# TheaQG/DiffusionModelsCustom

Measured on NVIDIA B200. Metric: samples_per_s_T1000_ddpm_sampling, higher is better.
Workload: dtype fp16 operands, fp32 accumulate (fp32 state/update)

## Files before the change

### diffusionmodelscustom_b200/_native.py

```python
from __future__ import annotations

import ctypes as C
import os

_PKG = os.path.dirname(os.path.abspath(__file__))
LIB_PATH = os.environ.get("B2D_LIB") or os.path.join(_PKG, "libb200ddpm.so")

FAMILY_R, FAMILY_D = 0, 1
INTERP_MODES = {"bicubic": 0, "bilinear": 1, "nearest": 2}

SYMBOLS = ["b2d_last_error", "b2d_abi_version", "b2d_create", "b2d_destroy", "b2d_load_weights", "b2d_set_schedule",
           "b2d_set_conditioning", "b2d_forward", "b2d_sample", "b2d_sample_host", "b2d_last_launch_count", "b2d_debug_read", "b2d_profile_step",
           "b2d_op_conv2d", "b2d_op_layernorm", "b2d_op_attention", "b2d_op_attn_block", "b2d_op_attn_block_out", "b2d_op_instnorm", "b2d_op_posterior_update", "b2d_saturation_count", "b2d_debug_attn_trace", "b2d_ensemble_run",
           "b2d_op_noise_image", "b2d_op_weighted_mse", "b2d_op_eval_daily", "b2d_op_eval_pixel", "b2d_op_histogram", "b2d_encoder_forward", "b2d_decoder_forward", "b2d_op_final_layer",
           "b2d_set_timesteps", "b2d_op_ddim_update"]


class Config(C.Structure):
    _fields_ = [(n, C.c_int32) for n in ("family", "img_size", "max_batch", "c_hr", "c_out", "has_lsm", "has_topo",
                                         "cond_channels", "num_classes", "n_heads", "attn_ff", "debug_simt_conv",
                                         "interp_mode", "stem_embedding")]


class Tensor(C.Structure):
    _fields_ = [("name", C.c_char_p), ("data", C.c_void_p), ("ndim", C.c_int32), ("shape", C.c_int64 * 4)]


class OpProfile(C.Structure):
    _fields_ = [("name", C.c_char * 48), ("klass", C.c_char * 24), ("flops", C.c_double), ("bytes", C.c_double),
                ("ms", C.c_double)]


class NativeError(RuntimeError):
    pass


_lib = None


def lib():
    global _lib
    if _lib is None:
        if not os.path.exists(LIB_PATH):
            raise NativeError(f"{LIB_PATH} is missing: build it with `python -m diffusionmodelscustom_b200.build` "
                              "(there is no fallback path)")
        L = C.CDLL(LIB_PATH)
        L.b2d_last_error.restype = C.c_char_p
        L.b2d_abi_version.restype = C.c_int
        L.b2d_create.argtypes = [C.POINTER(Config), C.POINTER(C.c_void_p)]
        L.b2d_destroy.argtypes = [C.c_void_p]
        L.b2d_destroy.restype = None
        L.b2d_load_weights.argtypes = [C.c_void_p, C.POINTER(Tensor), C.c_int32]
        L.b2d_set_schedule.argtypes = [C.c_void_p, C.c_void_p, C.c_void_p, C.c_void_p, C.c_int32]
        L.b2d_set_conditioning.argtypes = [C.c_void_p, C.c_void_p, C.c_void_p, C.c_void_p, C.c_int32, C.c_int32,
                                           C.c_void_p, C.c_int32, C.c_void_p]
        L.b2d_forward.argtypes = [C.c_void_p, C.c_void_p, C.c_void_p, C.c_void_p, C.c_int32, C.c_void_p]
        L.b2d_sample.argtypes = [C.c_void_p, C.c_void_p, C.c_void_p, C.c_uint64, C.c_uint64, C.c_float, C.c_int32,
                                 C.c_void_p]
        L.b2d_sample_host.argtypes = [C.c_void_p, C.c_void_p, C.c_void_p, C.c_void_p, C.c_void_p, C.c_int32, C.c_int32,
                                      C.c_void_p, C.c_void_p, C.c_uint64, C.c_uint64, C.c_float, C.c_int32]
        L.b2d_last_launch_count.argtypes = [C.c_void_p]
        L.b2d_last_launch_count.restype = C.c_int64
        L.b2d_debug_read.argtypes = [C.c_void_p, C.c_char_p, C.c_void_p, C.c_int64, C.POINTER(C.c_int32), C.POINTER(C.c_int32)]
        L.b2d_profile_step.argtypes = [C.c_void_p, C.c_void_p, C.c_void_p, C.c_int32, C.c_int32, C.POINTER(OpProfile),
                                       C.c_int32, C.POINTER(C.c_int32)]
        L.b2d_op_conv2d.argtypes = [C.c_void_p] * 5 + [C.c_int32, C.c_void_p] + [C.c_int32] * 12 + [C.c_void_p]
        L.b2d_op_layernorm.argtypes = [C.c_void_p] * 4 + [C.c_int32, C.c_int32, C.c_void_p]
        L.b2d_op_attention.argtypes = [C.c_void_p, C.c_void_p] + [C.c_int32] * 4 + [C.c_void_p]
        L.b2d_op_attn_block.argtypes = [C.c_void_p] * 5 + [C.c_int32] * 4 + [C.c_void_p]
        L.b2d_op_attn_block_out.argtypes = [C.c_void_p] * 7 + [C.c_int32] * 5 + [C.c_void_p]
        L.b2d_op_instnorm.argtypes = [C.c_void_p, C.c_void_p, C.c_void_p, C.c_int32, C.c_void_p, C.c_void_p] + \
                                     [C.c_int32] * 3 + [C.c_void_p]
        L.b2d_op_final_layer.argtypes = [C.c_void_p] * 4 + [C.c_int32] * 4 + [C.c_void_p]
        L.b2d_op_posterior_update.argtypes = [C.c_void_p] * 6 + [C.c_int32, C.c_int32, C.c_int64, C.c_uint64, C.c_uint64,
                                                                 C.c_float, C.c_void_p]
        L.b2d_set_timesteps.argtypes = [C.c_void_p, C.c_void_p, C.c_int32, C.c_float]
        L.b2d_op_ddim_update.argtypes = [C.c_void_p] * 4 + [C.c_int32] * 3 + [C.c_float, C.c_int32, C.c_int64, C.c_uint64,
                                                              C.c_uint64, C.c_float, C.c_void_p]
        L.b2d_op_noise_image.argtypes = [C.c_void_p] * 6 + [C.c_int32, C.c_int64, C.c_uint64, C.c_uint64, C.c_float, C.c_void_p]
        L.b2d_op_weighted_mse.argtypes = [C.c_void_p] * 3 + [C.c_float, C.c_float, C.c_void_p, C.c_int64, C.c_void_p]
        L.b2d_op_eval_daily.argtypes = [C.c_void_p] * 4 + [C.c_int32, C.c_int64, C.c_void_p]
        L.b2d_op_eval_pixel.argtypes = [C.c_void_p] * 5 + [C.c_int32, C.c_int64, C.c_void_p]
        L.b2d_op_histogram.argtypes = [C.c_void_p, C.c_int64, C.c_float, C.c_float, C.c_int32, C.c_void_p, C.c_void_p]
        L.b2d_encoder_forward.argtypes = [C.c_void_p, C.c_void_p, C.c_void_p, C.POINTER(C.c_void_p), C.c_int32, C.c_void_p]
        L.b2d_decoder_forward.argtypes = [C.c_void_p, C.POINTER(C.c_void_p), C.c_void_p, C.c_void_p, C.c_int32, C.c_void_p]
        L.b2d_saturation_count.argtypes = [C.c_int32]
        L.b2d_saturation_count.restype = C.c_uint32
        if L.b2d_abi_version() != 1:
            raise NativeError("libb200ddpm.so ABI version mismatch")
        _lib = L
    return _lib


def check(rc: int):
    if rc != 0:
        raise NativeError(f"b200ddpm error {rc}: {lib().b2d_last_error().decode(errors='replace')}")


def ptr(t):
    return None if t is None else t.data_ptr()
```

### diffusionmodelscustom_b200/csrc/b200ddpm.cu

```cuda
#include "../../include/b200ddpm.h"

#include <chrono>
#include <cmath>
#include <cstring>
#include <functional>
#include <map>
#include <memory>
#include <vector>

#include "attention.cuh"
#include "attention_tc.cuh"
#include "attention_tc2.cuh"
#include "attention_tc3.cuh"
#include "attention_tc3d32.cuh"
#include "attention_tc6.cuh"
#include "attention_tc8.cuh"
#include "attn_block.cuh"
#include "common.cuh"
#include "conv.cuh"
#include "conv_persist.cuh"
#include "elementwise.cuh"
#include "evalops.cuh"
#include "gemm_stream.cuh"
#include "norm_fused.cuh"
#include "tail_tc.cuh"

namespace b2d {
thread_local Status g_status;
int g_pdl_enabled = getenv("B2D_NO_PDL") ? 0 : 1;

static inline cudaStream_t as_stream(void* s) { return reinterpret_cast<cudaStream_t>(s); }

struct HostTensor {
    std::vector<float> v;
    std::vector<int64_t> shape;
    size_t numel() const { return v.size(); }
};

static inline uint16_t f2h(float f) {
    const float c = f > 65504.0f ? 65504.0f : (f < -65504.0f ? -65504.0f : f);
    const __half h = __float2half_rn(c);
    uint16_t u;
    memcpy(&u, &h, 2);
    return u;
}

typedef std::function<int(cudaStream_t)> OpFn;
struct Op {
    std::string name;
    std::string klass;
    double flops = 0;
    double bytes = 0;
    OpFn fn;
    bool side = false;
    bool join = false;
    int operator()(cudaStream_t st) const { return fn(st); }
};
struct OpList {
    std::vector<Op> v;
    Op pending;
    void meta(const std::string& name, const std::string& klass, double flops, double bytes) {
        pending.name = name; pending.klass = klass; pending.flops = flops; pending.bytes = bytes;
    }
    void push_back(OpFn f) {
        pending.fn = std::move(f);
        v.push_back(pending);
        pending = Op();
    }
};

struct EnsembleRes;
void ensemble_release(EnsembleRes* r);
struct Handle {
    b2d_config cfg{};
    int num_sms = 148;
    std::vector<void*> allocs;
    std::vector<void*> prog_allocs;
    bool in_prog = false;
// ... 642 lines not shown
        const std::string r0 = "l" + std::to_string(li) + "b0", r1 = "l" + std::to_string(li) + "b1";
        f16* t1 = bd.act(n_out);
        f16* b0 = bd.act(n_out);
        f16* pre = bd.act(n_out);
        const f16* identity = cur;
        const int stride = (li > 1) ? 2 : 1;
        if (li > 1) {
            f16* ds = bd.act(n_out);
            ops.pending.side = true;
            bd.conv(cur, hin, hin, cin, ds, cout, 1, 2, 0, false, r0 + ".ds", nullptr, nullptr, 0, 0);
            identity = ds;
        }
        bd.conv(cur, hin, hin, cin, t1, cout, 3, stride, 1, false, r0 + ".c1", nullptr, nullptr, 0, 1);
        ops.pending.join = (li > 1);
        bd.conv(t1, hout, hout, cout, b0, cout, 3, 1, 1, false, r0 + ".c2", identity, nullptr, 0, 1);
        bd.conv(b0, hout, hout, cout, t1, cout, 3, 1, 1, false, r1 + ".c1", nullptr, nullptr, 0, 1);
        bd.conv(t1, hout, hout, cout, pre, cout, 3, 1, 1, false, r1 + ".c2", b0, temb + TEMB_ENC_OFF[li], TS, 1);
        fmap[li] = bd.act(n_out);
        bd.attention(pre, hout, cout, "ea" + std::to_string(li), fmap[li], 0);
        h->taps["pre" + std::to_string(li + 1)] = {pre, cout, hout};
        h->taps["fmap" + std::to_string(li + 1)] = {fmap[li], cout, hout};
        cur = fmap[li];
        cin = cout;
    }
    h->dec_begin_op = (int)ops.v.size();
    for (int i = 0; i < 5; ++i) h->fmaps[i] = {fmap[i], ENC_CH[i], s[i + 1]};
    const f16* dcur = fmap[4];
    for (int i = 0; i < 4; ++i) {
        const int ci = DEC_IN[i], co = DEC_OUT[i];
        const int hin = s[5 - i], hout = s[4 - i];
        const std::string r = "d" + std::to_string(i);
        f16* up = bd.act((size_t)B * hout * hout * ci);
        bd.conv(dcur, hin, hin, ci, up, ci, 1, 1, 0, true, r + ".up", nullptr, nullptr, 0, 0);
        if (!bd.instnorm_fused(up, nullptr, nullptr, 0, up, hout, ci)) {
            float* st1 = bd.stats_slice(ci);
            bd.plane_stats(up, hout, ci, st1);
            bd.instnorm_apply(up, st1, nullptr, nullptr, 0, up, hout, ci);
        }
        f16* cv = bd.act((size_t)B * hout * hout * co);
        bd.conv(up, hout, hout, ci, cv, co, 3, 1, 1, false, r + ".conv", nullptr, nullptr, 0, 0);
        f16* pre = bd.act((size_t)B * hout * hout * co);
        if (!bd.instnorm_fused(cv, fmap[3 - i], temb + TEMB_DEC_OFF[i], TS, pre, hout, co)) {
            float* st2 = bd.stats_slice(co);
            bd.plane_stats(cv, hout, co, st2);
            bd.instnorm_apply(cv, st2, fmap[3 - i], temb + TEMB_DEC_OFF[i], TS, pre, hout, co);
        }
        f16* dout = bd.act((size_t)B * hout * hout * co);
        bd.attention(pre, hout, co, "da" + std::to_string(i), dout, 1 );
        h->taps["dec" + std::to_string(i) + "_pre"] = {pre, co, hout};
        h->taps["dec" + std::to_string(i)] = {dout, co, hout};
        dcur = dout;
    }
    h->temb_free_op = (int)ops.v.size();
    {
        f16* up = bd.act((size_t)B * H * H * 64);
        bd.conv(dcur, s[1], s[1], 64, up, 64, 1, 1, 0, true, "final.up", nullptr, nullptr, 0, 0);
        float* st = bd.stats_slice(64);
        bd.plane_stats(up, H, 64, st);
        Handle* hh = h;
        const float* tw = bd.W<float>("tail.w");
        const float* tb = bd.W<float>("tail.b");
        const float* twk = bd.W<float>("tail.wk");
        const int cout = c.c_out, Hh = H;
        ops.meta("final.conv", "tail_conv", 2.0 * B * Hh * Hh * 576 * cout, (double)B * Hh * Hh * (64 * 2 + 4 * cout));
        static const bool no_tc_tail = getenv("B2D_NO_TC_TAIL") != nullptr;
        auto ttp = std::make_shared<TailTcPlan>();
        const bool tc_tail = tail_tc_supported(Hh, Hh, cout) && !no_tc_tail;
        if (tc_tail && tail_tc_plan_build(*ttp, up, B, Hh, Hh) != 0) return g_status.code ? g_status.code : fail(-1, "tail plan failed");
        ops.push_back([=](cudaStream_t s2) {
            dim3 grid((Hh + 31) / 32, (Hh + 7) / 8, B);
            static const bool simt_tail = getenv("B2D_SIMT_TAIL") != nullptr;
            if (tc_tail)
                return tail_tc_launch(*ttp, st, twk, tb, hh->cur_eps, Hh, Hh, s2);
            if (cout <= 8 && !simt_tail)
                B2D_CUDA(launch_k(tail_mma_kernel, dim3(grid), dim3(256), TAILM_SMEM, s2, up, st, twk, tb, hh->cur_eps, Hh, Hh, cout));
            else
                B2D_CUDA(launch_k(tail_conv_kernel, dim3(grid), dim3(256), TAIL_SMEM, s2, up, st, tw, tb, hh->cur_eps, Hh, Hh, cout));
            B2D_CUDA(cudaGetLastError());
            return 0;
        });
    }
    if (bd.err) return g_status.code ? g_status.code : fail(-1, "program build failed");
    if (h->stats_floats > STATS_CAPACITY_PER_SAMPLE * (size_t)c.max_batch) return fail(-1, "internal: stats buffer too small");
    h->step_ops.swap(ops.v);
    h->prog_B = B;
    return 0;
}

template <typename K>
static int set_carveout(K kern) {
    B2D_CUDA(cudaFuncSetAttribute(kern, cudaFuncAttributePreferredSharedMemoryCarveout, cudaSharedmemCarveoutMaxShared));
    return 0;
}
static int init_uniform_carveout() {
    static bool done = false;
    if (done || getenv("B2D_NO_CARVEOUT")) return 0;
    B2D_TRY(set_carveout(conv_tc_kernel<64, 4>));
    B2D_TRY(set_carveout(conv_tc_kernel<64, 8>));
    B2D_TRY(set_carveout(conv_tc_kernel<128, 3>));
    B2D_TRY(set_carveout(conv_tc_kernel<128, 6>));
    B2D_TRY(set_carveout(conv_simt_kernel));
    B2D_TRY(set_carveout(layernorm_rows_kernel<64>));
    B2D_TRY(set_carveout(layernorm_rows_kernel<128>));
    B2D_TRY(set_carveout(layernorm_rows_kernel<256>));
    B2D_TRY(set_carveout(layernorm_rows_kernel<512>));
    B2D_TRY(set_carveout(flash_attn_kernel<16>));
    B2D_TRY(set_carveout(flash_attn_kernel<32>));
    B2D_TRY(set_carveout(flash_attn_kernel<64>));
    B2D_TRY(set_carveout(flash_attn_kernel<128>));
    B2D_TRY(set_carveout(attn_small_d_kernel<2>));
    B2D_TRY(set_carveout(attn_small_d_kernel<4>));
    B2D_TRY(set_carveout(attn_small_d_kernel<8>));
    B2D_TRY(set_carveout(attn_tc_kernel));
    B2D_TRY(set_carveout(attn_tc2_kernel<0>));
    B2D_TRY(set_carveout(attn_tc2_kernel<1>));
    B2D_TRY(set_carveout(attn_tc2_kernel<2>));
    B2D_TRY(set_carveout(attn_tc2_kernel<3>));
    B2D_TRY(set_carveout(attn_tc2_kernel<4>));
// ... 136 lines not shown
        B2D_TRY(h->alloc(&h->d_ddim_coef, T + 1));
        h->ddim_cap = T + 1;
    }
    std::vector<int> tau(h->ddim_tau);
    tau.resize(S + 2, 0);
    std::vector<float4> coef(S);
    for (int k = 0; k < S; ++k)
        coef[k] = ddim_coefficients(h->h_alpha_hat[tau[k]], k + 1 < S ? h->h_alpha_hat[tau[k + 1]] : 1.0f, h->ddim_eta);
    B2D_CUDA(cudaMemcpy(h->d_ddim_tau, tau.data(), tau.size() * sizeof(int), cudaMemcpyHostToDevice));
    B2D_CUDA(cudaMemcpy(h->d_ddim_coef, coef.data(), coef.size() * sizeof(float4), cudaMemcpyHostToDevice));
    h->ddim_dirty = false;
    return 0;
}

}

using namespace b2d;

extern "C" {

const char* b2d_last_error(void) { return g_status.msg.c_str(); }
int b2d_abi_version(void) { return B2D_ABI_VERSION; }

int b2d_create(const b2d_config* cfg, b2d_handle** out) {
    B2D_CHECK(cfg && out, "null argument");
    B2D_CHECK(cfg->family == B2D_FAMILY_R || cfg->family == B2D_FAMILY_D, "unknown family");
    B2D_CHECK(is_pow2(cfg->img_size) && cfg->img_size >= 32 && cfg->img_size <= 128, "img_size must be 32, 64 or 128");
    B2D_CHECK(cfg->max_batch >= 1, "max_batch must be positive");
    B2D_CHECK(cfg->c_hr >= 1 && cfg->c_out >= 1, "channel counts must be positive");
    int dev = 0, ndev = 0;
    cudaError_t e = cudaGetDeviceCount(&ndev);
    if (e != cudaSuccess || ndev == 0)
        return fail(-2, "no CUDA device: this library has no CPU fallback (" + std::string(cudaGetErrorString(e)) + ")");
    B2D_CUDA(cudaGetDevice(&dev));
    cudaDeviceProp prop;
    B2D_CUDA(cudaGetDeviceProperties(&prop, dev));
    B2D_CHECK(prop.major == 10, "b200ddpm kernels are compiled for sm_100a only");
    auto* h = new b2d_handle();
    h->cfg = *cfg;
    if (h->cfg.n_heads <= 0) h->cfg.n_heads = 4;
    h->num_sms = prop.multiProcessorCount;
    int rc = 0;
    do {
        if ((rc = conv_tc_init_attrs())) break;
        if ((rc = conv_tcp_init_attrs())) break;
        if ((rc = flash_attn_init_attrs())) break;
        if ((rc = attn_tc_init_attrs())) break;
        if ((rc = attn_tc2_init_attrs())) break;
        if ((rc = attn_tc3_init_attrs())) break;
        if ((rc = attn_tc5_init_attrs())) break;
        if ((rc = attn_tc6_init_attrs())) break;
        if ((rc = attn_tc8_init_attrs())) break;
        if ((rc = tail_tc_init_attrs())) break;
        if ((rc = gemm_stream_init_attrs())) break;
        if ((rc = attn_block_init_attrs())) break;
        if ((rc = norm_fused_init_attrs())) break;
        if ((rc = init_uniform_carveout())) break;
        const int B = cfg->max_batch, H = cfg->img_size;
        const size_t n = (size_t)B * cfg->c_hr * H * H, plane = (size_t)H * H;
        if ((rc = init_batch_buffers(h))) break;
        if ((rc = h->alloc(&h->d_x_work, n))) break;
        if ((rc = h->alloc(&h->d_job, 1))) break;
        if (cfg->family == B2D_FAMILY_R) {
            if (cfg->has_lsm && (rc = h->alloc(&h->d_lsm_stage, (size_t)B * plane))) break;
            if (cfg->has_topo && (rc = h->alloc(&h->d_topo_stage, (size_t)B * plane))) break;
        }
        h->cond_stage_elems = (size_t)B * std::max(cfg->cond_channels, 1) * plane;
        if ((rc = h->alloc(&h->d_cond_stage, h->cond_stage_elems))) break;
        if (cudaMallocHost(reinterpret_cast<void**>(&h->h_y_pinned), (size_t)B * sizeof(int)) != cudaSuccess) {
            rc = fail(-2, "pinned label staging allocation failed");
            break;
        }
    } while (0);
    if (rc) {
        delete h;
        return rc;
    }
    *out = h;
    return 0;
}

void b2d_destroy(b2d_handle* h) { delete h; }

int b2d_load_weights(b2d_handle* h, const b2d_tensor* tensors, int32_t n) {
    B2D_CHECK(h && tensors && n > 0, "null argument");
    B2D_CHECK(!h->weights_loaded, "weights already loaded on this handle (create a new handle to reload)");
    h->sd.clear();
    for (int i = 0; i < n; ++i) {
        const b2d_tensor& t = tensors[i];
        B2D_CHECK(t.name && t.data && t.ndim >= 0 && t.ndim <= 4, "malformed tensor entry");
        HostTensor ht;
        size_t numel = 1;
        for (int d = 0; d < t.ndim; ++d) {
            ht.shape.push_back(t.shape[d]);
            numel *= (size_t)t.shape[d];
        }
        ht.v.assign(t.data, t.data + numel);
        h->sd[t.name] = std::move(ht);
    }
    int rc = (h->cfg.family == B2D_FAMILY_R) ? pack_family_r(h) : pack_family_d(h);
    h->sd.clear();
    if (rc) return rc;
    h->weights_loaded = true;
    return 0;
}

// ... 543 lines not shown
    float* stats = ws;
    float* partial = ws + n_stats;
    unsigned int* counters = reinterpret_cast<unsigned int*>(ws + n_stats + n_part);
    cudaMemsetAsync(counters, 0, n_cnt * 4, st);
    dim3 grid(nslab, ngrp, B);
    B2D_CUDA(launch_k(plane_stats_kernel, dim3(grid), dim3(256), 0, st, (const f16*)x, partial, counters, stats, HW, C, 256));
    const size_t total8 = (size_t)B * HW * C / 8;
    const int blocks = (int)std::min<size_t>((total8 + 255) / 256, (size_t)148 * 16);
    B2D_CUDA(launch_k(instnorm_apply_kernel, dim3(blocks), dim3(256), 0, st, (const f16*)x, stats, (const f16*)skip, vec, vec_stride, (f16*)y, HW, C,
                                                  total8));
    cudaError_t e = cudaGetLastError();
    cudaStreamSynchronize(st);
    cudaFree(ws);
    B2D_CUDA(e);
    return 0;
}

int b2d_op_final_layer(const void* x, const float* w, const float* bias, float* out, int32_t B, int32_t H, int32_t W,
                       int32_t use_mma_sync, void* stream) {
    cudaStream_t st = as_stream(stream);
    B2D_CHECK(x && w && bias && out && B >= 1 && H >= 1 && W >= 1, "bad argument");
    const int HW = H * W, C = 64;
    const int nslab = (HW + 255) / 256;
    float* ws = nullptr;
    const size_t n_stats = (size_t)B * C * 2, n_part = (size_t)B * nslab * 128, n_cnt = (size_t)B;
    B2D_CUDA(cudaMalloc(&ws, (n_stats + n_part + n_cnt) * 4));
    float* stats = ws;
    float* partial = ws + n_stats;
    unsigned int* counters = reinterpret_cast<unsigned int*>(ws + n_stats + n_part);
    cudaMemsetAsync(counters, 0, n_cnt * 4, st);
    int rc = 0;
    do {
        cudaError_t e = launch_k(plane_stats_kernel, dim3(nslab, 1, B), dim3(256), 0, st, (const f16*)x, partial, counters, stats, HW, C, 256);
        if (e != cudaSuccess) { rc = fail(-2, cudaGetErrorString(e)); break; }
        if (!use_mma_sync && tail_tc_supported(H, W, 1)) {
            if ((rc = tail_tc_init_attrs())) break;
            TailTcPlan pl;
            if ((rc = tail_tc_plan_build(pl, (const f16*)x, B, H, W))) break;
            rc = tail_tc_launch(pl, stats, w, bias, out, H, W, st);
        } else {
            e = cudaFuncSetAttribute(tail_mma_kernel, cudaFuncAttributeMaxDynamicSharedMemorySize, TAILM_SMEM);
            if (e == cudaSuccess)
                e = launch_k(tail_mma_kernel, dim3((W + 31) / 32, (H + 7) / 8, B), dim3(256), TAILM_SMEM, st, (const f16*)x, stats, w, bias, out, H, W, 1);
            if (e != cudaSuccess) rc = fail(-2, cudaGetErrorString(e));
        }
    } while (0);
    cudaError_t e2 = cudaStreamSynchronize(st);
    cudaFree(ws);
    if (rc) return rc;
    B2D_CUDA(e2);
    return 0;
}

int b2d_op_posterior_update(float* x, const float* eps, const float* z, const float* betas, const float* alphas,
                            const float* alpha_hat, int32_t i, int32_t B, int64_t per_sample, uint64_t seed,
                            uint64_t sample_offset, float noise_scale, void* stream) {
    B2D_CHECK(x && eps && betas && alphas && alpha_hat && B >= 1 && per_sample >= 1, "bad argument");
    B2D_CHECK(per_sample % 4 == 0, "per-sample element count must be a multiple of 4 (vectorised update)");
    cudaStream_t st = as_stream(stream);
    struct Scratch { int* step = nullptr; SampleJob* job = nullptr; };
    static thread_local Scratch sc;
    if (!sc.step) {
        B2D_CUDA(cudaMalloc(&sc.step, 16));
        B2D_CUDA(cudaMalloc(&sc.job, sizeof(SampleJob)));
    }
    const size_t n = (size_t)B * per_sample;
    SampleJob job{};
    job.noise = z ? z - (size_t)i * n : nullptr;
    job.seed = seed;
    job.sample_offset = sample_offset;
    job.noise_stride = n;
    job.noise_scale = noise_scale;
    B2D_CUDA(launch_k(set_job_kernel, dim3(1), dim3(32), 0, st, sc.job, job, sc.step + 2, sc.step, (int)i, 0));
    const int blocks = (int)std::min<size_t>((n / 4 + 255) / 256, (size_t)148 * 8);
    B2D_CUDA(launch_k(posterior_update_kernel, dim3(blocks), dim3(256), 0, st, x, eps, sc.job, alphas, betas, alpha_hat, sc.step, nullptr, B, n,
                      (size_t)per_sample));
    B2D_CUDA(cudaGetLastError());
    return 0;
}

int b2d_op_ddim_update(float* x, const float* eps, const float* z_or_null, const float* alpha_hat, int32_t T, int32_t t,
                       int32_t t_prev, float eta, int32_t B, int64_t per_sample, uint64_t seed, uint64_t sample_offset,
                       float noise_scale, void* stream) {
    B2D_CHECK(x && eps && alpha_hat && B >= 1 && per_sample >= 1 && T >= 2, "bad argument");
    B2D_CHECK(per_sample % 4 == 0, "per-sample element count must be a multiple of 4 (vectorised update)");
    B2D_CHECK(t >= 1 && t <= T - 1, "t must lie in [1, T-1]");
    B2D_CHECK(t_prev == -1 || (t_prev >= 1 && t_prev < t), "t_prev must be -1 (final step) or lie in [1, t-1]");
    B2D_CHECK(eta >= 0.f && eta <= 1.f, "eta must lie in [0, 1]");
    cudaStream_t st = as_stream(stream);
    float ah[2] = {0.f, 1.f};
    B2D_CUDA(cudaMemcpyAsync(&ah[0], alpha_hat + t, 4, cudaMemcpyDeviceToHost, st));
    if (t_prev >= 1) B2D_CUDA(cudaMemcpyAsync(&ah[1], alpha_hat + t_prev, 4, cudaMemcpyDeviceToHost, st));
    B2D_CUDA(cudaStreamSynchronize(st));
    const float4 c = ddim_coefficients(ah[0], ah[1], eta);
    struct Scratch { int* step = nullptr; SampleJob* job = nullptr; int* tau = nullptr; float4* coef = nullptr; };
    static thread_local Scratch sc;
    if (!sc.step) {
        B2D_CUDA(cudaMalloc(&sc.step, 16));
        B2D_CUDA(cudaMalloc(&sc.job, sizeof(SampleJob)));
        B2D_CUDA(cudaMalloc(&sc.tau, 16));
        B2D_CUDA(cudaMalloc(&sc.coef, sizeof(float4)));
    }
    const size_t n = (size_t)B * per_sample;
    SampleJob job{};
    job.noise = z_or_null;
    job.seed = seed;
// ... 85 lines not shown
```

### include/b200ddpm.h

```cpp
#ifndef B200DDPM_H
#define B200DDPM_H

#include <stddef.h>
#include <stdint.h>

#ifdef __cplusplus
extern "C" {
#endif

#define B2D_ABI_VERSION 1

typedef struct b2d_handle b2d_handle;

enum { B2D_FAMILY_R = 0,
       B2D_FAMILY_D = 1   };

typedef struct b2d_config {
    int32_t family;
    int32_t img_size;
    int32_t max_batch;
    int32_t c_hr;
    int32_t c_out;
    int32_t has_lsm;
    int32_t has_topo;
// ... 60 lines not shown
typedef struct b2d_ensemble_stats {
    int32_t sub_batches;
    int32_t out_pinned;
    int64_t launches;
    double gather_ms;
    double wall_ms;
} b2d_ensemble_stats;
int b2d_ensemble_run(b2d_handle* h, const b2d_ensemble_job* job, b2d_ensemble_stats* stats);

unsigned int b2d_saturation_count(int32_t reset);

int64_t b2d_last_launch_count(const b2d_handle* h);
typedef struct b2d_op_profile {
    char name[48];
    char klass[24];
    double flops;
    double bytes;
    double ms;
} b2d_op_profile;
int b2d_profile_step(b2d_handle* h, const float* x, const int64_t* t_host, int32_t B, int32_t reps, b2d_op_profile* out,
                     int32_t max_ops, int32_t* n_ops);

int b2d_debug_read(b2d_handle* h, const char* name, float* out_host, int64_t max_elems, int32_t* C_out, int32_t* hw_out);

int b2d_op_noise_image(const float* x0, const int64_t* t_dev, const float* alpha_hat, const float* noise_or_null, float* x_t,
                       float* noise_out, int32_t B, int64_t per_sample, uint64_t seed, uint64_t sample_offset, float noise_scale,
                       void* stream);
int b2d_op_weighted_mse(const float* input, const float* target, const float* sdf_or_null, float max_land_weight,
                        float min_sea_weight, float* out_scalar_dev, int64_t n, void* stream);
int b2d_op_eval_daily(const float* gen, const float* eval, float* mae_out, float* rmse_out, int32_t n_samples, int64_t hw,
                      void* stream);
int b2d_op_eval_pixel(const float* gen, const float* eval, float* mae_out, float* rmse_out, float* bias_out, int32_t n_samples,
                      int64_t hw, void* stream);
int b2d_op_histogram(const float* x, int64_t n, float lo, float hi, int32_t bins, unsigned long long* counts_dev, void* stream);

int b2d_debug_attn_trace(long long* out_host, int32_t max_elems);

int b2d_op_conv2d(const void* in_f16, const void* w_packed_f16, const float* bias, const void* residual_f16,
                  const float* post_add, int32_t post_stride, void* out_f16, int32_t B, int32_t Hi, int32_t Wi,
                  int32_t Cin, int32_t Cout, int32_t R, int32_t S, int32_t stride, int32_t pad, int32_t convt,
                  int32_t act, int32_t impl, void* stream);
int b2d_op_layernorm(const void* x_f16, const float* gamma, const float* beta, void* y_f16, int32_t rows, int32_t C,
                     void* stream);
int b2d_op_attention(const void* qkv_f16, void* o_f16, int32_t B, int32_t L, int32_t C, int32_t heads, void* stream);
int b2d_op_attn_block(const void* x_f16, const void* w_folded_f16, const float* c1, const float* bias, void* o_f16,
                      int32_t B, int32_t L, int32_t C, int32_t heads, void* stream);
int b2d_op_attn_block_out(const void* x_f16, const void* w_folded_f16, const float* c1, const float* bias, const void* wo_f16,
                          const float* out_bias, void* y_f16, int32_t B, int32_t L, int32_t C, int32_t heads,
                          int32_t final_act, void* stream);
int b2d_op_instnorm(const void* x_f16, const void* skip_f16, const float* vec, int32_t vec_stride, void* y_f16,
                    float* stats_ws, int32_t B, int32_t HW, int32_t C, void* stream);
int b2d_op_final_layer(const void* x_f16, const float* w_kmajor, const float* bias, float* out, int32_t B, int32_t H, int32_t W,
                       int32_t use_mma_sync, void* stream);
int b2d_op_posterior_update(float* x, const float* eps, const float* z_or_null, const float* betas, const float* alphas,
                            const float* alpha_hat, int32_t i, int32_t B, int64_t per_sample, uint64_t seed,
                            uint64_t sample_offset, float noise_scale, void* stream);

#ifdef __cplusplus
}
#endif
#endif
```

Before: 26.31.

## Fuse final transposed conv, instance-norm stats and 3x3 tail conv into tcgen05 kernels

Replaces the final 2x-upsampling transposed conv, the instance-norm statistics and the 3x3 output conv with two warp-specialised TMA/tcgen05 kernels. The first pass recomputes the upsampled activations per tile in TMEM and reduces per-channel mean and variance across CTAs using atomic counters. The second pass recomputes them, folds the normalisation into the tail weights and applies the 3x3 stencil from shared-memory slots. This avoids writing and reading back the full-resolution 64-channel fp16 intermediate, at the cost of doing the transposed-conv GEMM twice plus halo tiles and cross-block synchronisation.

After: 26.82, median of 6. 1.9% higher.

```diff
diff --git a/diffusionmodelscustom_b200/_native.py b/diffusionmodelscustom_b200/_native.py
--- a/diffusionmodelscustom_b200/_native.py
+++ b/diffusionmodelscustom_b200/_native.py
@@ -13,6 +13,7 @@
            "b2d_set_conditioning", "b2d_forward", "b2d_sample", "b2d_sample_host", "b2d_last_launch_count", "b2d_debug_read", "b2d_profile_step",
            "b2d_op_conv2d", "b2d_op_layernorm", "b2d_op_attention", "b2d_op_attn_block", "b2d_op_attn_block_out", "b2d_op_instnorm", "b2d_op_posterior_update", "b2d_saturation_count", "b2d_debug_attn_trace", "b2d_ensemble_run",
            "b2d_op_noise_image", "b2d_op_weighted_mse", "b2d_op_eval_daily", "b2d_op_eval_pixel", "b2d_op_histogram", "b2d_encoder_forward", "b2d_decoder_forward", "b2d_op_final_layer",
+           "b2d_op_final_layer_convt",
            "b2d_set_timesteps", "b2d_op_ddim_update"]
 
 
@@ -72,6 +73,7 @@
         L.b2d_op_instnorm.argtypes = [C.c_void_p, C.c_void_p, C.c_void_p, C.c_int32, C.c_void_p, C.c_void_p] + \
                                      [C.c_int32] * 3 + [C.c_void_p]
         L.b2d_op_final_layer.argtypes = [C.c_void_p] * 4 + [C.c_int32] * 4 + [C.c_void_p]
+        L.b2d_op_final_layer_convt.argtypes = [C.c_void_p] * 6 + [C.c_int32] * 3 + [C.c_void_p]
         L.b2d_op_posterior_update.argtypes = [C.c_void_p] * 6 + [C.c_int32, C.c_int32, C.c_int64, C.c_uint64, C.c_uint64,
                                                                  C.c_float, C.c_void_p]
         L.b2d_set_timesteps.argtypes = [C.c_void_p, C.c_void_p, C.c_int32, C.c_float]
diff --git a/diffusionmodelscustom_b200/csrc/b200ddpm.cu b/diffusionmodelscustom_b200/csrc/b200ddpm.cu
--- a/diffusionmodelscustom_b200/csrc/b200ddpm.cu
+++ b/diffusionmodelscustom_b200/csrc/b200ddpm.cu
@@ -24,6 +24,7 @@
 #include "gemm_stream.cuh"
 #include "norm_fused.cuh"
 #include "tail_tc.cuh"
+#include "final_tc.cuh"
 
 namespace b2d {
 thread_local Status g_status;
@@ -772,7 +773,29 @@
         dcur = dout;
     }
     h->temb_free_op = (int)ops.v.size();
-    {
+    static const bool no_tc_tail = getenv("B2D_NO_TC_TAIL") != nullptr;
+    if (final_tc_supported(H, H, c.c_out) && !no_tc_tail && !c.debug_simt_conv) {
+        float* st = bd.stats_slice(64);
+        float* ws = nullptr;
+        if (h->alloc(&ws, final_tc_ws_floats(B, H, H)) != 0) return fail(-2, "final layer workspace");
+        auto fp = std::make_shared<FinalTcPlan>();
+        if (final_tc_plan_build(*fp, dcur, bd.W<f16>("final.up.w"), bd.W<float>("final.up.b"), bd.W<float>("tail.wk"), bd.W<float>("tail.b"),
+                                st, ws, nullptr, B, H, H, h->num_sms) != 0)
+            return g_status.code ? g_status.code : fail(-1, "final layer plan failed");
+        if (cudaMemset(fp->a.counters, 0, (size_t)B * sizeof(unsigned int)) != cudaSuccess) return fail(-2, "final layer counters");
+        const double in_px = (double)B * s[1] * s[1], convt_flops = 2.0 * in_px * 64 * 256;
+        ops.meta("final.stats", "final_stats", convt_flops, in_px * 64 * 2 + 4.0 * B * 64 * 2);
+        ops.push_back([fp](cudaStream_t st2) { return final_tc_launch_stats(*fp, st2); });
+        const double loads_px = (double)fp->loads1 * 128;
+        ops.meta("final.conv", "final_tc", 2.0 * loads_px * 64 * 256 + 2.0 * loads_px * 4 * 64 * 16,
+                 loads_px * 64 * 2 + (double)B * H * H * 4);
+        Handle* hh = h;
+        ops.push_back([fp, hh](cudaStream_t st2) {
+            FinalTcPlan pl = *fp;
+            pl.a.out = hh->cur_eps;
+            return final_tc_launch_apply(pl, st2);
+        });
+    } else {
         f16* up = bd.act((size_t)B * H * H * 64);
         bd.conv(dcur, s[1], s[1], 64, up, 64, 1, 1, 0, true, "final.up", nullptr, nullptr, 0, 0);
         float* st = bd.stats_slice(64);
@@ -783,7 +806,6 @@
         const float* twk = bd.W<float>("tail.wk");
         const int cout = c.c_out, Hh = H;
         ops.meta("final.conv", "tail_conv", 2.0 * B * Hh * Hh * 576 * cout, (double)B * Hh * Hh * (64 * 2 + 4 * cout));
-        static const bool no_tc_tail = getenv("B2D_NO_TC_TAIL") != nullptr;
         auto ttp = std::make_shared<TailTcPlan>();
         const bool tc_tail = tail_tc_supported(Hh, Hh, cout) && !no_tc_tail;
         if (tc_tail && tail_tc_plan_build(*ttp, up, B, Hh, Hh) != 0) return g_status.code ? g_status.code : fail(-1, "tail plan failed");
@@ -1026,6 +1048,7 @@
         if ((rc = attn_tc6_init_attrs())) break;
         if ((rc = attn_tc8_init_attrs())) break;
         if ((rc = tail_tc_init_attrs())) break;
+        if ((rc = final_tc_init_attrs())) break;
         if ((rc = gemm_stream_init_attrs())) break;
         if ((rc = attn_block_init_attrs())) break;
         if ((rc = norm_fused_init_attrs())) break;
@@ -1675,6 +1698,34 @@
     return 0;
 }
 
+int b2d_op_final_layer_convt(const void* x, const void* wt, const float* bt, const float* w, const float* bias, float* out, int32_t B,
+                             int32_t H, int32_t W, void* stream) {
+    cudaStream_t st = as_stream(stream);
+    B2D_CHECK(x && wt && bt && w && bias && out && B >= 1, "bad argument");
+    B2D_CHECK(final_tc_supported(H, W, 1), "final layer shape not supported (W a power of two in [4, 128], (H/2 * W/2) % 128 == 0)");
+    int dev = 0, sms = 148;
+    cudaGetDevice(&dev);
+    cudaDeviceGetAttribute(&sms, cudaDevAttrMultiProcessorCount, dev);
+    float* ws = nullptr;
+    const size_t n_stats = (size_t)B * 64 * 2, n_ws = final_tc_ws_floats(B, H, W);
+    B2D_CUDA(cudaMalloc(&ws, (n_stats + n_ws) * 4));
+    int rc = 0;
+    do {
+        FinalTcPlan pl;
+        if ((rc = final_tc_init_attrs())) break;
+        if ((rc = final_tc_plan_build(pl, (const f16*)x, (const f16*)wt, bt, w, bias, ws, ws + n_stats, out, B, H, W, sms))) break;
+        cudaError_t e = cudaMemsetAsync(pl.a.counters, 0, (size_t)B * sizeof(unsigned int), st);
+        if (e != cudaSuccess) { rc = fail(-2, cudaGetErrorString(e)); break; }
+        if ((rc = final_tc_launch_stats(pl, st))) break;
+        rc = final_tc_launch_apply(pl, st);
+    } while (0);
+    cudaError_t e2 = cudaStreamSynchronize(st);
+    cudaFree(ws);
+    if (rc) return rc;
+    B2D_CUDA(e2);
+    return 0;
+}
+
 int b2d_op_posterior_update(float* x, const float* eps, const float* z, const float* betas, const float* alphas,
                             const float* alpha_hat, int32_t i, int32_t B, int64_t per_sample, uint64_t seed,
                             uint64_t sample_offset, float noise_scale, void* stream) {
diff --git a/diffusionmodelscustom_b200/csrc/final_tc.cuh b/diffusionmodelscustom_b200/csrc/final_tc.cuh
--- /dev/null
+++ b/diffusionmodelscustom_b200/csrc/final_tc.cuh
@@ -0,0 +1,444 @@
+#pragma once
+#include "common.cuh"
+#include "conv.cuh"
+
+#ifndef FTX_KSTEPS
+#define FTX_KSTEPS 4
+#endif
+#ifndef FTX_NOCOL
+#define FTX_NOCOL 0
+#endif
+namespace b2d {
+
+__device__ __forceinline__ void tma_prefetch_l2_2d(const void* desc, int c0, int c1) {
+    asm volatile("cp.async.bulk.prefetch.tensor.2d.L2.global.tile [%0, {%1, %2}];" ::"l"((uint64_t)desc), "r"(c0), "r"(c1) : "memory");
+}
+
+constexpr int FT_EPI_WARPS = 16;
+constexpr int FT_EPI_THREADS = FT_EPI_WARPS * 32;
+constexpr int FT_THREADS = 64 + FT_EPI_THREADS;
+constexpr int FT_Y_BYTES = 4 * CONV_A_BYTES;
+constexpr int FT_SLOTS = 4;
+constexpr int FT_PSTRIDE = 9 * 128 + 16;
+constexpr int FT_SLOT_FLOATS = 4 * FT_PSTRIDE;
+constexpr int FT_PREFETCH = 6;
+template <int PASS>
+__host__ __device__ constexpr int ft_stages() { return PASS == 0 ? 4 : 3; }
+template <int PASS>
+__host__ __device__ constexpr int ft_smem_bytes() {
+    return 1024 + ft_stages<PASS>() * CONV_A_BYTES + 256 * 128 +
+           (PASS == 0 ? 2 * FT_Y_BYTES : FT_Y_BYTES + 2048 + FT_SLOTS * FT_SLOT_FLOATS * 4) + 256;
+}
+
+struct FinalTcArgs {
+    const float* bt;
+    const float* wk;
+    const float* bias;
+    float* stats;
+    float* partial;
+    unsigned int* counters;
+    float* out;
+    int B, h, w;
+    int band_tiles;
+};
+
+template <int PASS>
+__global__ void __launch_bounds__(FT_THREADS, 1)
+    final_tc_kernel(const __grid_constant__ CUtensorMap tmX,
+                    const __grid_constant__ CUtensorMap tmW,
+                    const FinalTcArgs a) {
+    pdl_launch_dependents();
+    constexpr int FT_STAGES = ft_stages<PASS>();
+    extern __shared__ uint8_t ft_raw[];
+    uint8_t* smem = reinterpret_cast<uint8_t*>((reinterpret_cast<uintptr_t>(ft_raw) + 1023) & ~uintptr_t(1023));
+    uint8_t* sX = smem;
+    uint8_t* sWt = sX + FT_STAGES * CONV_A_BYTES;
+    uint8_t* sY = sWt + 256 * 128;
+    uint8_t* sW1 = sY + FT_Y_BYTES;
+    float* sT = reinterpret_cast<float*>(sW1 + 2048);
+    uint64_t* bars = reinterpret_cast<uint64_t*>(PASS == 0 ? sY + 2 * FT_Y_BYTES : reinterpret_cast<uint8_t*>(sT + FT_SLOTS * FT_SLOT_FLOATS));
+    uint64_t* x_full = bars;
+    uint64_t* x_empty = bars + FT_STAGES;
+    uint64_t* w_full = bars + 2 * FT_STAGES;
+    uint64_t* t_full = w_full + 1;
+    uint64_t* t_empty = t_full + 2;
+    uint64_t* y_full = t_empty + 2;
+    uint64_t* t2_full = y_full + 1;
+    uint32_t* tmem_slot = reinterpret_cast<uint32_t*>(t2_full + 1);
+    __shared__ __align__(16) float s_bias[256];
+    __shared__ float s_st[128];
+    __shared__ float s_k[9];
+    __shared__ int s_last;
+
+    const int warp = threadIdx.x >> 5, lane = threadIdx.x & 31;
+    const int tpi = (a.h * a.w) >> 7;
+    int first, nload, b = 0, t0 = 0, nt = 0, lo = 0;
+    if (PASS == 0) {
+        const long long total = (long long)a.B * tpi;
+        first = (int)((long long)blockIdx.x * total / gridDim.x);
+        nload = (int)((long long)(blockIdx.x + 1) * total / gridDim.x) - first;
+    } else {
+        b = blockIdx.y;
+        t0 = blockIdx.x * a.band_tiles;
+        nt = min(a.band_tiles, tpi - t0);
+        lo = t0 > 0 ? t0 - 1 : t0;
+        nload = min(t0 + nt + 1, tpi) - lo;
+        first = b * tpi + lo;
+    }
+
+    if (warp == 0 && lane == 0) {
+        tma_prefetch_desc(&tmX);
+        tma_prefetch_desc(&tmW);
+    }
+    if (warp == 1) {
+        if (lane == 0) {
+            for (int i = 0; i < FT_STAGES; ++i) { mbar_init(&x_full[i], 1); mbar_init(&x_empty[i], 1); }
+            mbar_init(w_full, 1);
+            for (int i = 0; i < 2; ++i) { mbar_init(&t_full[i], 1); mbar_init(&t_empty[i], FT_EPI_WARPS); }
+            mbar_init(y_full, FT_EPI_WARPS);
+            mbar_init(t2_full, 1);
+            fence_mbar_init();
+        }
+        __syncwarp();
+        tmem_alloc(tmem_slot, 512);
+        tmem_relinquish();
+    }
+    pdl_wait();
+    if (threadIdx.x < 256) s_bias[threadIdx.x] = __ldg(a.bt + (threadIdx.x & 63));
+    if (PASS == 1) {
+        if (threadIdx.x < 128) s_st[threadIdx.x] = a.stats[(size_t)b * 128 + threadIdx.x];
+        __syncthreads();
+        for (int i = threadIdx.x; i < 16 * 8; i += FT_THREADS) {
+            const int n = i >> 3, j = i & 7;
+            uint4 v = make_uint4(0u, 0u, 0u, 0u);
+            if (n < 9) {
+                float f[8];
+#pragma unroll
+                for (int e = 0; e < 8; ++e) f[e] = __ldg(a.wk + n * 64 + j * 8 + e) * s_st[2 * (j * 8 + e) + 1];
+                v.x = pack_h2(f[0], f[1]); v.y = pack_h2(f[2], f[3]); v.z = pack_h2(f[4], f[5]); v.w = pack_h2(f[6], f[7]);
+            }
+            *reinterpret_cast<uint4*>(sW1 + n * 128 + ((j ^ (n & 7)) << 4)) = v;
+        }
+        if (warp < 9) {
+            const float* wr = a.wk + warp * 64;
+            float m = __ldg(wr + lane) * s_st[2 * lane + 1] * s_st[2 * lane] +
+                      __ldg(wr + lane + 32) * s_st[2 * (lane + 32) + 1] * s_st[2 * (lane + 32)];
+            m = warp_sum(m);
+            if (lane == 0) s_k[warp] = m;
+        }
+        fence_proxy_async();
+    }
+    tc_fence_before();
+    __syncthreads();
+    tc_fence_after();
+    const uint32_t tmem = *tmem_slot;
+
+    if (warp == 0) {
+        if (elect_one()) {
+            mbar_arrive_expect_tx(w_full, 256 * 128);
+            tma_load_2d(sWt, &tmW, w_full, 0, 0);
+        }
+        if (elect_one())
+            for (int i = FT_STAGES; i < FT_PREFETCH && i < nload; ++i) tma_prefetch_l2_2d(&tmX, 0, (first + i) * 128);
+        __syncwarp();
+        for (int i = 0; i < nload; ++i) {
+            const int st = i % FT_STAGES;
+            if (i + FT_PREFETCH < nload && elect_one()) tma_prefetch_l2_2d(&tmX, 0, (first + i + FT_PREFETCH) * 128);
+            __syncwarp();
+            mbar_wait(&x_empty[st], ((i / FT_STAGES) & 1) ^ 1);
+            if (elect_one()) {
+                mbar_arrive_expect_tx(&x_full[st], CONV_A_BYTES);
+                tma_load_2d(sX + st * CONV_A_BYTES, &tmX, &x_full[st], 0, (first + i) * 128);
+            }
+            __syncwarp();
+        }
+    } else if (warp == 1) {
+        constexpr uint32_t idesc_y = umma_idesc_f16(128, 256);
+        constexpr uint32_t idesc_t = umma_idesc_f16(128, 16);
+        const uint64_t dw = umma_desc_sw128(smem_u32(sWt));
+        const uint64_t dw1 = umma_desc_sw128(smem_u32(sW1));
+        mbar_wait(w_full, 0);
+        auto mma_y = [&](int i) {
+            const int st = i % FT_STAGES, acc = i & 1;
+            mbar_wait(&t_empty[acc], ((i >> 1) & 1) ^ 1);
+            mbar_wait(&x_full[st], (i / FT_STAGES) & 1);
+            tc_fence_after();
+            if (elect_one()) {
+                const uint64_t da = umma_desc_sw128(smem_u32(sX + st * CONV_A_BYTES));
+#pragma unroll
+                for (int k = 0; k < FTX_KSTEPS; ++k) umma_f16(tmem + acc * 256, da + (uint64_t)(k * 2), dw + (uint64_t)(k * 2), idesc_y, k != 0);
+                umma_commit(&x_empty[st]);
+                umma_commit(&t_full[acc]);
+            }
+            __syncwarp();
+        };
+        if (PASS == 0) {
+            for (int i = 0; i < nload; ++i) mma_y(i);
+        } else {
+            if (nload > 0) mma_y(0);
+            for (int i = 0; i < nload; ++i) {
+                if (i + 1 < nload) mma_y(i + 1);
+                mbar_wait(y_full, i & 1);
+                tc_fence_after();
+                if (elect_one()) {
+#pragma unroll
+                    for (int ph = 0; ph < 4; ++ph) {
+                        const uint64_t da = umma_desc_sw128(smem_u32(sY + ph * CONV_A_BYTES));
+#pragma unroll
+                        for (int k = 0; k < 4; ++k)
+                            umma_f16(tmem + (i & 1) * 256 + ph * 16, da + (uint64_t)(k * 2), dw1 + (uint64_t)(k * 2), idesc_t, k != 0);
+                    }
+                    umma_commit(t2_full);
+                }
+                __syncwarp();
+            }
+        }
+    } else {
+        const int e = threadIdx.x - 64;
+        const int q = warp & 3, g = (warp - 2) >> 2;
+        const int row = q * 32 + lane, sw = row & 7;
+        float s[8], s2[8];
+#pragma unroll
+        for (int j = 0; j < 8; ++j) { s[j] = 0.f; s2[j] = 0.f; }
+        float kk[9];
+        float bias0 = 0.f;
+        if (PASS == 1) {
+#pragma unroll
+            for (int t = 0; t < 9; ++t) kk[t] = s_k[t];
+            bias0 = __ldg(a.bias);
+        }
+        const int lw = 31 - __clz(a.w);
+        const int Wo = 2 * a.w, Ho = 2 * a.h, lW = lw + 1;
+        auto drain = [&](int i, auto&& overlap) {
+            const int acc = i & 1;
+            uint8_t* yb = sY + (PASS == 0 ? (i & 1) * FT_Y_BYTES : 0);
+            mbar_wait(&t_full[acc], (i >> 1) & 1);
+            tc_fence_after();
+            float satm = 0.f;
+            uint4* yrow = reinterpret_cast<uint4*>(yb + g * CONV_A_BYTES + row * 128);
+#pragma unroll
+            for (int hf = 0; hf < 2; ++hf) {
+                uint32_t v[32];
+                tmem_ld32(tmem + ((uint32_t)(q * 32) << 16) + (uint32_t)(acc * 256 + g * 64 + hf * 32), v);
+                if (hf == 0) overlap();
+                tmem_ld_wait();
+#pragma unroll
+                for (int jj = 0; jj < 4; ++jj) {
+                    const int j = hf * 4 + jj;
+                    const float4 b0 = *reinterpret_cast<const float4*>(&s_bias[g * 64 + j * 8]);
+                    const float4 b1 = *reinterpret_cast<const float4*>(&s_bias[g * 64 + j * 8 + 4]);
+                    uint4 o;
+                    o.x = pack_h2_acc(__uint_as_float(v[jj * 8 + 0]) + b0.x, __uint_as_float(v[jj * 8 + 1]) + b0.y, satm);
+                    o.y = pack_h2_acc(__uint_as_float(v[jj * 8 + 2]) + b0.z, __uint_as_float(v[jj * 8 + 3]) + b0.w, satm);
+                    o.z = pack_h2_acc(__uint_as_float(v[jj * 8 + 4]) + b1.x, __uint_as_float(v[jj * 8 + 5]) + b1.y, satm);
+                    o.w = pack_h2_acc(__uint_as_float(v[jj * 8 + 6]) + b1.z, __uint_as_float(v[jj * 8 + 7]) + b1.w, satm);
+                    yrow[j ^ sw] = o;
+                }
+            }
+            tc_fence_before();
+            if (PASS == 0) {
+                __syncwarp();
+                if (lane == 0) mbar_arrive(&t_empty[acc]);
+            }
+            return satm;
+        };
+        if (PASS == 0) {
+            const int j = e & 31, rg = e >> 5;
+            auto colsum = [&](int i) {
+                if (FTX_NOCOL) return;
+                const uint8_t* col = sY + (i & 1) * FT_Y_BYTES + (j >> 3) * CONV_A_BYTES + rg * 8 * 128;
+#pragma unroll
+                for (int rr = 0; rr < 8; ++rr) {
+                    const uint4 u = *reinterpret_cast<const uint4*>(col + rr * 128 + (((j & 7) ^ rr) << 4));
+                    const uint32_t uu[4] = {u.x, u.y, u.z, u.w};
+#pragma unroll
+                    for (int p = 0; p < 4; ++p) {
+                        const float2 t = unpack_h2(uu[p]);
+                        s[2 * p] += t.x; s[2 * p + 1] += t.y;
+                        s2[2 * p] = fmaf(t.x, t.x, s2[2 * p]); s2[2 * p + 1] = fmaf(t.y, t.y, s2[2 * p + 1]);
+                    }
+                }
+            };
+            for (int i = 0; i <= nload; ++i) {
+                if (i < nload)
+                    drain(i, [&] { if (i > 0) colsum(i - 1); });
+                else
+                    colsum(i - 1);
+                named_bar_sync(1, FT_EPI_THREADS);
+                if (i == 0) continue;
+                const int tile = first + i - 1;
+                if ((tile + 1) % tpi != 0 && i != nload) continue;
+                float* red = reinterpret_cast<float*>(sY + ((i - 1) & 1) * FT_Y_BYTES);
+                float4* r4 = reinterpret_cast<float4*>(red + rg * 256 + j * 8);
+                r4[0] = make_float4(s[0], s[1], s[2], s[3]);
+                r4[1] = make_float4(s[4], s[5], s[6], s[7]);
+                r4 = reinterpret_cast<float4*>(red + 4096 + rg * 256 + j * 8);
+                r4[0] = make_float4(s2[0], s2[1], s2[2], s2[3]);
+                r4[1] = make_float4(s2[4], s2[5], s2[6], s2[7]);
+#pragma unroll
+                for (int c = 0; c < 8; ++c) { s[c] = 0.f; s2[c] = 0.f; }
+                named_bar_sync(1, FT_EPI_THREADS);
+                const int bb = tile / tpi;
+                const long long total = (long long)a.B * tpi;
+                auto owner = [&](long long t) { return (int)(((t + 1) * gridDim.x - 1) / total); };
+                const int c_first = owner((long long)bb * tpi), nparts = owner((long long)(bb + 1) * tpi - 1) - c_first + 1;
+                float* part = a.partial + (size_t)bb * tpi * 128;
+                if (e < 64) {
+                    float S = 0.f, Q = 0.f;
+#pragma unroll
+                    for (int ph = 0; ph < 4; ++ph)
+#pragma unroll
+                        for (int r = 0; r < 16; ++r) { S += red[r * 256 + ph * 64 + e]; Q += red[4096 + r * 256 + ph * 64 + e]; }
+                    float* pp = part + (size_t)(blockIdx.x - c_first) * 128;
+                    pp[e] = S;
+                    pp[64 + e] = Q;
+                    __threadfence();
+                }
+                named_bar_sync(1, FT_EPI_THREADS);
+                if (e == 0) s_last = atomicAdd(&a.counters[bb], 1u) == (unsigned)(nparts - 1);
+                named_bar_sync(1, FT_EPI_THREADS);
+                if (s_last) {
+                    __threadfence();
+                    if (e < 64) {
+                        float S = 0.f, Q = 0.f;
+                        for (int k = 0; k < nparts; ++k) { S += __ldcg(part + (size_t)k * 128 + e); Q += __ldcg(part + (size_t)k * 128 + 64 + e); }
+                        const float inv = 1.0f / (float)(4 * a.h * a.w);
+                        const float mean = S * inv;
+                        const float var = fmaxf(Q * inv - mean * mean, 0.f);
+                        float* sto = a.stats + ((size_t)bb * 64 + e) * 2;
+                        sto[0] = mean;
+                        sto[1] = rsqrtf(var + 1e-5f);
+                    }
+                    if (e == 0) a.counters[bb] = 0u;
+                }
+            }
+        } else {
+            auto stencil = [&](int o) {
+                const int tile = lo + o;
+                if (o < 0 || tile < t0 || tile >= t0 + nt) return;
+                const int i0 = (tile * 128) >> lw;
+                const int y = 2 * i0 + (e >> lW), x = e & (Wo - 1);
+                float acc_o = bias0;
+#pragma unroll
+                for (int r = 0; r < 3; ++r) {
+                    const int yy = y + r - 1;
+                    if (yy < 0 || yy >= Ho) continue;
+#pragma unroll
+                    for (int c = 0; c < 3; ++c) {
+                        const int xx = x + c - 1;
+                        if (xx < 0 || xx >= Wo) continue;
+                        const int qs = ((yy >> 1) << lw) + (xx >> 1);
+                        const int so = (qs >> 7) - lo;
+                        const int ph = ((yy & 1) << 1) | (xx & 1);
+                        acc_o += sT[(so % FT_SLOTS) * FT_SLOT_FLOATS + ph * FT_PSTRIDE + (r * 3 + c) * 128 + (qs & 127)];
+                    }
+                }
+                a.out[(size_t)b * Ho * Wo + (size_t)2 * i0 * Wo + e] = acc_o;
+            };
+            for (int i = 0; i < nload; ++i) {
+                float satm = drain(i, [] {});
+                const int tile_i = lo + i;
+                if (tile_i >= t0 && tile_i < t0 + nt) sat_flush(satm);
+                fence_proxy_async();
+                __syncwarp();
+                if (lane == 0) mbar_arrive(y_full);
+                if (i >= 2) stencil(i - 2);
+                mbar_wait(t2_full, i & 1);
+                tc_fence_after();
+                uint32_t tv[16];
+                asm volatile(
+                    "tcgen05.ld.sync.aligned.32x32b.x16.b32 {%0, %1, %2, %3, %4, %5, %6, %7, %8, %9, %10, %11, %12, %13, %14, %15}, [%16];"
+                    : "=r"(tv[0]), "=r"(tv[1]), "=r"(tv[2]), "=r"(tv[3]), "=r"(tv[4]), "=r"(tv[5]), "=r"(tv[6]), "=r"(tv[7]), "=r"(tv[8]),
+                      "=r"(tv[9]), "=r"(tv[10]), "=r"(tv[11]), "=r"(tv[12]), "=r"(tv[13]), "=r"(tv[14]), "=r"(tv[15])
+                    : "r"(tmem + ((uint32_t)(q * 32) << 16) + (uint32_t)((i & 1) * 256 + g * 16))
+                    : "memory");
+                tmem_ld_wait();
+                tc_fence_before();
+                __syncwarp();
+                if (lane == 0) mbar_arrive(&t_empty[i & 1]);
+                float* slot = sT + (i % FT_SLOTS) * FT_SLOT_FLOATS + g * FT_PSTRIDE;
+#pragma unroll
+                for (int t = 0; t < 9; ++t) slot[t * 128 + row] = __uint_as_float(tv[t]) - kk[t];
+                named_bar_sync(1, FT_EPI_THREADS);
+            }
+            stencil(nload - 2);
+            stencil(nload - 1);
+        }
+    }
+    tc_fence_before();
+    __syncthreads();
+    if (warp == 1) {
+        tc_fence_after();
+        tmem_dealloc(tmem, 512);
+    }
+}
+
+struct FinalTcPlan {
+    CUtensorMap tmX, tmW;
+    FinalTcArgs a;
+    dim3 grid0, grid1;
+    int loads1 = 0;
+};
+
+inline bool final_tc_supported(int H, int W, int c_out) {
+    return c_out == 1 && H >= 2 && H % 2 == 0 && is_pow2(W) && W >= 4 && W <= 128 && ((H / 2) * (W / 2)) % 128 == 0;
+}
+
+inline size_t final_tc_ws_floats(int B, int H, int W) { return (size_t)B * ((H / 2) * (W / 2) / 128) * 128 + B; }
+
+inline int final_tc_plan_build(FinalTcPlan& pl, const f16* x, const f16* wt, const float* bt, const float* w, const float* bias,
+                               float* stats, float* ws, float* out, int B, int H, int W, int num_sms) {
+    B2D_CHECK(final_tc_supported(H, W, 1), "final layer shape not supported by the fused kernel");
+    const int h = H / 2, wi = W / 2, tpi = h * wi / 128;
+    uint64_t dx[2] = {64, (uint64_t)B * h * wi};
+    uint64_t sx[1] = {128};
+    uint32_t bx[2] = {64, 128};
+    B2D_TRY(make_tmap_f16(&pl.tmX, x, 2, dx, sx, bx));
+    uint64_t dw[2] = {64, 256};
+    uint32_t bw[2] = {64, 256};
+    B2D_TRY(make_tmap_f16(&pl.tmW, wt, 2, dw, sx, bw));
+    FinalTcArgs& a = pl.a;
+    a.bt = bt; a.wk = w; a.bias = bias; a.stats = stats; a.out = out;
+    a.partial = ws;
+    a.counters = reinterpret_cast<unsigned int*>(ws + (size_t)B * tpi * 128);
+    a.B = B; a.h = h; a.w = wi;
+    const int total = B * tpi;
+    pl.grid0 = dim3(total < num_sms ? total : num_sms, 1, 1);
+    int best = tpi;
+    long long best_cost = -1;
+    for (int band = tpi; band >= 1; --band) {
+        const int nb = (tpi + band - 1) / band;
+        const long long waves = ((long long)nb * B + num_sms - 1) / num_sms;
+        const long long cost = waves * (band + (nb > 1 ? (nb > 2 ? 2 : 1) : 0));
+        if (best_cost < 0 || cost < best_cost) { best_cost = cost; best = band; }
+    }
+    a.band_tiles = best;
+    const int nb = (tpi + best - 1) / best;
+    pl.grid1 = dim3(nb, B, 1);
+    pl.loads1 = 0;
+    for (int k = 0; k < nb; ++k) {
+        const int t0 = k * best, nt = std::min(best, tpi - t0);
+        pl.loads1 += std::min(t0 + nt + 1, tpi) - (t0 > 0 ? t0 - 1 : t0);
+    }
+    pl.loads1 *= B;
+    return 0;
+}
+
+inline int final_tc_init_attrs() {
+    B2D_CUDA(cudaFuncSetAttribute(final_tc_kernel<0>, cudaFuncAttributeMaxDynamicSharedMemorySize, ft_smem_bytes<0>()));
+    B2D_CUDA(cudaFuncSetAttribute(final_tc_kernel<1>, cudaFuncAttributeMaxDynamicSharedMemorySize, ft_smem_bytes<1>()));
+    B2D_CUDA(cudaFuncSetAttribute(final_tc_kernel<0>, cudaFuncAttributePreferredSharedMemoryCarveout, cudaSharedmemCarveoutMaxShared));
+    B2D_CUDA(cudaFuncSetAttribute(final_tc_kernel<1>, cudaFuncAttributePreferredSharedMemoryCarveout, cudaSharedmemCarveoutMaxShared));
+    return 0;
+}
+
+inline int final_tc_launch_stats(const FinalTcPlan& pl, cudaStream_t st) {
+    B2D_CUDA(launch_k(final_tc_kernel<0>, pl.grid0, dim3(FT_THREADS), ft_smem_bytes<0>(), st, pl.tmX, pl.tmW, pl.a));
+    return 0;
+}
+inline int final_tc_launch_apply(const FinalTcPlan& pl, cudaStream_t st) {
+    B2D_CUDA(launch_k(final_tc_kernel<1>, pl.grid1, dim3(FT_THREADS), ft_smem_bytes<1>(), st, pl.tmX, pl.tmW, pl.a));
+    return 0;
+}
+
+}
diff --git a/include/b200ddpm.h b/include/b200ddpm.h
--- a/include/b200ddpm.h
+++ b/include/b200ddpm.h
@@ -136,6 +136,8 @@
                     float* stats_ws, int32_t B, int32_t HW, int32_t C, void* stream);
 int b2d_op_final_layer(const void* x_f16, const float* w_kmajor, const float* bias, float* out, int32_t B, int32_t H, int32_t W,
                        int32_t use_mma_sync, void* stream);
+int b2d_op_final_layer_convt(const void* x_f16, const void* wt_packed_f16, const float* bt, const float* w_kmajor, const float* bias,
+                             float* out, int32_t B, int32_t H, int32_t W, void* stream);
 int b2d_op_posterior_update(float* x, const float* eps, const float* z_or_null, const float* betas, const float* alphas,
                             const float* alpha_hat, int32_t i, int32_t B, int64_t per_sample, uint64_t seed,
                             uint64_t sample_offset, float noise_scale, void* stream);
```
